# One-2-3-45/One-2-3-45

Hardware: AMD Instinct MI355X
Metric: rays/sec + mesh-extract wall-clock per scene (8x256^2 views, 128^3 vol) (higher is better)
Workload: dtype f32 (matrix products as 3 f16 MFMAs on split operands, fp32 accumulate); 1 GPU; BASELINE config 2: 1 scene/GPU/step (a different seeded scene every step), 8 views 256x256, 128^3 volume, 262144 rays (64+64 samples), mesh grid 256^3; whole scene pass per step; views=8, volume=128, rays=262144, mesh_res=256, parallelism=scenes x1, precision=f16x3

## Files before the change

include/o2345.h:

```cpp
#ifndef O2345_H
#define O2345_H
#include <stddef.h>
#include <stdint.h>
#ifdef __cplusplus
extern "C" {
#endif

const char* o2345_last_error(void);
int o2345_version(void);
size_t o2345_render_io_size(void);
int o2345_render_io_layout(size_t* offsets_host, int n);
const char* o2345_knobs(void);

size_t o2345_costvol_workspace_bytes(int dx, int dy, int dz);
int o2345_costvol_index(const float* proj, int V, int H, int W, int dx, int dy, int dz, float voxel_size,
                        const float* origin_host, int min_views, uint8_t* cnt, int32_t* row_of_voxel, int32_t* coords,
                        int32_t* n_rows_dev, void* workspace, size_t workspace_bytes, void* stream);
int o2345_costvol_gather(const float* feats_nhwc, const float* proj, int V, int H, int W, int C, int dx, int dy, int dz,
                         float voxel_size, const float* origin_host, const uint8_t* cnt, const int32_t* coords,
                         int n_rows, float* out_rows, void* stream);
int o2345_nchw_to_nhwc(const float* in, float* out, int V, int C, int H, int W, void* stream);

int o2345_fpn_level(const float* fine, int c_in, const float* coarse, const float* weight, const float* bias, int V, int H, int W,
                    float* out, void* stream);
// ... 7 lines not shown
size_t o2345_conv2d_x3_weight_floats(int cin, int k);
int o2345_conv2d_pack_weights_x3(const float* w_oihw, int cout, int cin, int k, float* packed, void* stream);
int o2345_conv2d_x3(const float* in, int V, int cin, int Hi, int Wi, int in_pixel_stride, int in_channel_offset, const float* in_scale_shift, float slope,
                    const float* w_packed_x3, const float* bias, int cout, int k, int stride, float* out, const float* gamma, const float* beta, float eps,
                    int abs_gamma, float* out_scale_shift, void* workspace, size_t workspace_bytes, void* stream);
int o2345_fpn_level_act(const float* fine, const float* fine_scale_shift, float slope, int c_in, const float* coarse, const float* weight,
                        const float* bias, int V, int H, int W, float* out, void* stream);
int o2345_scale_shift_act(const float* x, int V, int C, int H, int W, const float* scale_shift, float slope, float* y_nchw, float* y_nhwc,
                          void* stream);
int o2345_visible_count_list(const float* proj, int V, int H, int W, float voxel_size, const float* origin_host,
                             const int32_t* coords, int n, uint8_t* cnt, void* stream);
int o2345_costvol_gather_list(const float* feats_nhwc, const float* proj, int V, int H, int W, int C, float voxel_size,
                              const float* origin_host, const uint8_t* cnt_row, const int32_t* coords, int n_rows,
                              float* out_rows, void* stream);
int o2345_build_index_grid(const int32_t* coords, int n, int ts, int nx, int ny, int nz, int32_t* grid, void* stream);
int o2345_prune_dilate(const float* sdf, const float* mask, int D, float threshold, int radius, uint8_t* out, void* stream);
int o2345_scatter_dense(const float* rows, const int32_t* row_of_voxel, int C, long long nvox, float* dense_cl,
                        float* dense_cf, float* mask, void* stream);

size_t o2345_sparse_downsample_workspace_bytes(int nxc, int nyc, int nzc);
int o2345_sparse_downsample(const int32_t* coords_fine, int n_fine, int ts, int nxc, int nyc, int nzc,
                            int32_t* row_of_cell, int32_t* coords_coarse, int32_t* n_coarse_dev, void* workspace,
                            size_t workspace_bytes, void* stream);
int o2345_sparse_conv3d(int mode, const float* in, int cin, const int32_t* in_grid, int gx, int gy, int gz,
                        const int32_t* out_coords, int n_out, int ts_out, const float* kernel, int cout, float* out,
                        void* stream);
int o2345_sparse_conv_x3_blob_floats(int cin, int cout);
int o2345_sparse_conv3d_x3(int mode, const float* in, int cin, const int32_t* in_grid, int gx, int gy, int gz,
                           const int32_t* out_coords, int n_out, int ts_out, const float* wblob, int cout, int identity_rows, float* out,
                           void* stream);
size_t o2345_bn_workspace_bytes(int C);
int o2345_bn_act_rows(const float* x, int n, int C, const float* gamma, const float* beta, float eps, float slope,
                      int abs_gamma, const float* skip, float* y, float* mean_var_out, void* workspace,
                      size_t workspace_bytes, void* stream);
size_t o2345_abn_workspace_bytes(int C);
int o2345_abn_nchw(const float* x, int V, int C, int H, int W, const float* gamma, const float* beta, float eps,
                   float slope, int abs_gamma, float* y_nchw, float* y_nhwc, void* workspace, size_t workspace_bytes,
                   void* stream);

int o2345_sdf_blob_floats(void);
int o2345_sdf_mlp(int variant, const float* blob, const float* vol_cl, int D, const float* pts, const int32_t* index,
                  const int32_t* n_dev, long long n, int grid_R, float sign, float* out_sdf, float* out_feat,
                  float* out_lat, float* out_grad, void* stream);
int o2345_sdf_mlp_ex(int variant, const float* blob, const float* vol_cl, int D, const float* pts, const int32_t* index,
                     const int32_t* n_dev, long long n, int grid_R, float sign, const float* lat_in, float* out_sdf,
                     float* out_feat, float* out_lat, float* out_grad, void* stream);
int o2345_sdf_mlp_x3(const float* blob, const float* vol_cl, int D, const float* pts, const int32_t* index, const int32_t* n_dev,
                     long long n, int grid_R, float sign, float* out_sdf, void* stream);
int o2345_sdf_grad_x3(const float* blob, const float* vol_cl, int D, const float* pts, const int32_t* index, const int32_t* n_dev,
                      long long n, int grid_R, float sign, float* out_sdf, float* out_grad, void* stream);
int o2345_sdf_grid_tables(const float* tab_axes, const float* bias_lane_order, int grid_R, float* tab_xy, void* stream);
int o2345_sdf_grid_x3(const float* blob, const float* vol_cl, int D, int grid_R, float sign, const float* tab_xy, const float* tab_z,
                      float* out_sdf, void* stream);

int o2345_ray_coarse(const float* rays_o, const float* rays_d, int R, float near, float far, int S, float* z, float* pts,
                     void* stream);
int o2345_ray_coarse_jitter(const float* rays_o, const float* rays_d, int R, float near, float far, int S,
                            const float* t_rand, float* z, float* pts, void* stream);
int o2345_ray_coarse_per_ray(const float* rays_o, const float* rays_d, int R, const float* near_ray, const float* far_ray, int S,
                             const float* t_rand, float* z, float* pts, void* stream);
int o2345_ray_upsample(const float* rays_o, const float* rays_d, int R, const float* z, const float* sdf, int S,
                       float inv_s, const float* maskvol, int D, float* wbuf, int n_imp, float* new_z, float* new_pts,
                       float* new_sdf, int32_t* list, int32_t* count_dev, void* stream);
int o2345_ray_merge(int R, float* z, float* sdf, int S, float* new_z, float* new_sdf, int n_new, void* stream);
int o2345_ray_finalize(const float* rays_o, const float* rays_d, int R, const float* z, int S, float sample_dist,
                       const float* maskvol, int D, float* mid_z, float* dists, float* pts, float* pm, float* sdf,
                       float* grad, float* rgb, int32_t* list, int32_t* count_dev, void* stream);
int o2345_ray_composite(const float* rays_o, const float* rays_d, int R, int S, const float* mid_z, const float* dists,
                        const float* pm, const float* sdf, const float* grad, const float* rgb, const uint8_t* nviews,
                        float inv_s, float alpha_inter_ratio, float background, float* color, float* depth,
                        float* weights, float* cdf, float* weights_sum, float* weights_max, float* depth_var,
                        float* alpha_sum, float* grad_err, uint8_t* color_mask, void* stream);

typedef struct O2345RenderIO {
    const float* sdf_blob;
    const float* color_x3_blob;
    const float* color_mfma_blob;
    const float* vol_cl;
    const float* maskvol;
    const float* cmaps;
    const float* proj;
    const float* cam_pos;
    int D, V, H, W;
    const float* rays_o; const float* rays_d;
    const float* near_ray;
    const float* far_ray;
    const float* query_cam;
    const float* t_rand;
    int R, n_samples, n_importance;
    int sdf_mode;
    int segment_rays;
    float near, far;
    float sample_dist;
    float inv_s, alpha_inter_ratio, background;
    float weight_cull;
    float* mid_z; float* dists; float* pm; float* sdf; float* grad; float* rgb; uint8_t* nviews;
    float* color; float* depth; float* weights; float* cdf; float* weights_sum; float* weights_max; float* depth_var;
    float* alpha_sum; float* grad_err; uint8_t* color_mask;
    float* z_vals;
    float* scalars;
    unsigned long long* color_stats;
} O2345RenderIO;
size_t o2345_list_sort_workspace_bytes(long long n_max, int V);
int o2345_list_sort_by_visibility(const float* pts, const int32_t* list, const int32_t* count_dev, long long n_max, const float* proj, int V, int H, int W,
                                  int32_t* list_out, uint32_t* keys_out, void* workspace, size_t workspace_bytes, void* stream);
size_t o2345_render_workspace_bytes(int R, int n_samples, int n_importance, int V);
// ... 92 lines not shown
```

one-2-3-45_amd/config.py:

```python
import os

PRECISIONS = ("f16x3", "fp32")
PRECISION = os.environ.get("O2345_PRECISION", "f16x3")
if PRECISION not in PRECISIONS:
    raise ValueError(f"O2345_PRECISION must be one of {PRECISIONS}, got {PRECISION!r}")


def sdf_precision(p=None):
    p = PRECISION if p is None else p
    if p not in PRECISIONS:
        raise ValueError(f"unknown precision {p!r}")
    return p


def color_precision(p=None):
    p = PRECISION if p is None else p
    if p not in PRECISIONS:
        raise ValueError(f"unknown precision {p!r}")
    return p


WEIGHT_CULL = float(os.environ.get("O2345_WEIGHT_CULL", "").strip() or 0.0) if "O2345_WEIGHT_CULL" in os.environ else 2.0 ** -24
if not (0.0 <= WEIGHT_CULL < 1.0):
    raise ValueError(f"O2345_WEIGHT_CULL must be in [0, 1), got {WEIGHT_CULL}")


def weight_cull(w=None):
    w = WEIGHT_CULL if w is None else float(w)
    if not (0.0 <= w < 1.0):
        raise ValueError(f"weight_cull must be in [0, 1), got {w}")
    return w


def warm_aten():
    return os.environ.get("O2345_WARM_ATEN", "1") not in ("", "0")


def prepack_resolutions():
    v = os.environ.get("O2345_PREPACK_RESOLUTIONS", "256")
    return tuple(int(x) for x in v.replace(",", " ").split())


def _non_negative_int(name, text):
    t = text.strip()
    if t == "":
        return 0
    if not t.isdigit():
        raise ValueError(f"{name} must be a non-negative integer, got {text!r}")
    return int(t)


MESH_MIN_COMPONENT_FACES = _non_negative_int("O2345_MESH_MIN_COMPONENT_FACES", os.environ.get("O2345_MESH_MIN_COMPONENT_FACES", ""))
MESH_KEEP_LARGEST = _non_negative_int("O2345_MESH_KEEP_LARGEST", os.environ.get("O2345_MESH_KEEP_LARGEST", "")) != 0


def mesh_min_component_faces(n=None):
    if n is None:
        return MESH_MIN_COMPONENT_FACES
    if isinstance(n, bool) or int(n) != n or n < 0:
        raise ValueError(f"min_component_faces must be a non-negative integer, got {n!r}")
    return int(n)


def mesh_keep_largest(k=None):
    return MESH_KEEP_LARGEST if k is None else bool(k)


def _finite_float(name, text, default, ok, what):
    t = text.strip()
    if t == "":
        return default
    try:
        x = float(t)
    except ValueError:
        x = float("nan")
    if not (x == x and abs(x) != float("inf") and ok(x)):
        raise ValueError(f"{name} must be {what}, got {text!r}")
    return x


MESH_SMOOTH_ITERATIONS = _non_negative_int("O2345_MESH_SMOOTH_ITERATIONS", os.environ.get("O2345_MESH_SMOOTH_ITERATIONS", ""))
MESH_SMOOTH_LAMBDA = _finite_float("O2345_MESH_SMOOTH_LAMBDA", os.environ.get("O2345_MESH_SMOOTH_LAMBDA", ""), 0.5, lambda x: 0.0 < x <= 1.0, "in (0, 1]")
MESH_SMOOTH_MU = _finite_float("O2345_MESH_SMOOTH_MU", os.environ.get("O2345_MESH_SMOOTH_MU", ""), -0.53, lambda x: x <= 0.0, "finite and <= 0")
_pin = os.environ.get("O2345_MESH_SMOOTH_PIN_BOUNDARY", "")
MESH_SMOOTH_PIN_BOUNDARY = True if _pin.strip() == "" else _non_negative_int("O2345_MESH_SMOOTH_PIN_BOUNDARY", _pin) != 0
del _pin


def mesh_smooth_iterations(n=None):
    if n is None:
        return MESH_SMOOTH_ITERATIONS
    if isinstance(n, bool) or int(n) != n or n < 0:
        raise ValueError(f"smooth_iterations must be a non-negative integer, got {n!r}")
    return int(n)


def mesh_smooth_lambda(lam=None):
    if lam is None:
        return MESH_SMOOTH_LAMBDA
    return _finite_float("lam", repr(float(lam)), None, lambda x: 0.0 < x <= 1.0, "in (0, 1]")


# ... 93 lines not shown
```

one-2-3-45_amd/csrc/geom_math.h:

```cpp
#pragma once
#include "common.h"

namespace o2345 {

O2345_HD void project_voxel(const float* __restrict__ P, float wx, float wy, float wz, int H, int W,
                            float& gx, float& gy, bool& valid) {
    float x = fmaf(P[2], wz, fmaf(P[1], wy, P[0] * wx)) + P[3];
    float y = fmaf(P[6], wz, fmaf(P[5], wy, P[4] * wx)) + P[7];
    float z = fmaf(P[10], wz, fmaf(P[9], wy, P[8] * wx)) + P[11];
    if (z >= 0.f) z = fmaxf(z, 1e-6f);
    gx = 2.f * (x / z) / (float)(W - 1) - 1.f;
    gy = 2.f * (y / z) / (float)(H - 1) - 1.f;
    valid = (fabsf(gx) <= 1.f) && (fabsf(gy) <= 1.f) && (z > 0.f);
}

struct Taps2D {
    int idx[4];
    float w[4];
};

O2345_HD Taps2D bilinear_taps(float gx, float gy, int H, int W) {
    Taps2D t;
    float ix = (gx + 1.f) / 2.f * (float)(W - 1);
    float iy = (gy + 1.f) / 2.f * (float)(H - 1);
    float x0 = floorf(ix), y0 = floorf(iy);
    float x1 = x0 + 1.f, y1 = y0 + 1.f;
    float wx1 = ix - x0, wx0 = x1 - ix, wy1 = iy - y0, wy0 = y1 - iy;
    bool bx0 = (x0 >= 0.f) && (x0 <= (float)(W - 1)), bx1 = (x1 >= 0.f) && (x1 <= (float)(W - 1));
    bool by0 = (y0 >= 0.f) && (y0 <= (float)(H - 1)), by1 = (y1 >= 0.f) && (y1 <= (float)(H - 1));
    int xi0 = (int)fminf(fmaxf(x0, 0.f), (float)(W - 1)), xi1 = (int)fminf(fmaxf(x1, 0.f), (float)(W - 1));
    int yi0 = (int)fminf(fmaxf(y0, 0.f), (float)(H - 1)), yi1 = (int)fminf(fmaxf(y1, 0.f), (float)(H - 1));
    t.idx[0] = yi0 * W + xi0; t.w[0] = (bx0 && by0) ? wx0 * wy0 : 0.f;
    t.idx[1] = yi0 * W + xi1; t.w[1] = (bx1 && by0) ? wx1 * wy0 : 0.f;
    t.idx[2] = yi1 * W + xi0; t.w[2] = (bx0 && by1) ? wx0 * wy1 : 0.f;
    t.idx[3] = yi1 * W + xi1; t.w[3] = (bx1 && by1) ? wx1 * wy1 : 0.f;
    return t;
}

struct Taps3D {
    int ix[2], iy[2], iz[2];
    float fx[2], fy[2], fz[2];
    bool ok;
};

O2345_HD Taps3D trilinear_ref_taps(float px, float py, float pz, int D) {
    Taps3D t;
    const float s = (float)(D - 1);
    float ix = (px + 1.f) / 2.f * s, iy = (py + 1.f) / 2.f * s, iz = (pz + 1.f) / 2.f * s;
    const float Df = (float)D;
    t.ok = (ix > 0.f) && (ix < Df) && (iy > 0.f) && (iy < Df) && (iz > 0.f) && (iz < Df);
    float x0 = floorf(ix), y0 = floorf(iy), z0 = floorf(iz);
    t.fx[0] = (x0 + 1.f) - ix; t.fx[1] = ix - x0;
    t.fy[0] = (y0 + 1.f) - iy; t.fy[1] = iy - y0;
    t.fz[0] = (z0 + 1.f) - iz; t.fz[1] = iz - z0;
    auto cl = [s](float v) { return (int)fminf(fmaxf(v, 0.f), s); };
    t.ix[0] = cl(x0); t.ix[1] = cl(x0 + 1.f);
    t.iy[0] = cl(y0); t.iy[1] = cl(y0 + 1.f);
    t.iz[0] = cl(z0); t.iz[1] = cl(z0 + 1.f);
    return t;
}

O2345_HD int nearest_index(float g, int D) {
    float i = nearbyintf(((g + 1.f) * (float)D - 1.f) / 2.f);
    return (i >= 0.f && i <= (float)(D - 1)) ? (int)i : -1;
}

O2345_HD int nearest_voxel(float px, float py, float pz, int D) {
    int x = nearest_index(px, D), y = nearest_index(py, D), z = nearest_index(pz, D);
    return (x < 0 || y < 0 || z < 0) ? -1 : (x * D + y) * D + z;
}

struct Axis2 {
    int i[2];
    float w[2];
};
O2345_HD Axis2 axis_taps_zeros(float g, int D) {
    Axis2 a;
    float s = (float)(D - 1);
    float f = (g + 1.f) / 2.f * s;
    float f0 = floorf(f), f1 = f0 + 1.f;
    a.w[0] = (f0 >= 0.f && f0 <= s) ? (f1 - f) : 0.f;
    a.w[1] = (f1 >= 0.f && f1 <= s) ? (f - f0) : 0.f;
    a.i[0] = (int)fminf(fmaxf(f0, 0.f), s);
    a.i[1] = (int)fminf(fmaxf(f1, 0.f), s);
    return a;
}

}
```

one-2-3-45_amd/csrc/sdf_common.h:

```cpp
#pragma once
#include "common.h"
#include "geom_math.h"
#include "pe_math.h"
#include "split_f16.h"

namespace o2345 {

constexpr int ST0 = 20;
constexpr int ST1 = 72;
constexpr int STB = 64;
constexpr int OFF_A0 = 0;
constexpr int OFF_A1 = OFF_A0 + 4 * ST0 * 64;
constexpr int OFF_A2 = OFF_A1 + 4 * ST1 * 64;
constexpr int OFF_A1T = OFF_A2 + 4 * ST1 * 64;
constexpr int OFF_A0T = OFF_A1T + 5 * STB * 64;
constexpr int OFF_MISC = OFF_A0T + 2 * STB * 64;
constexpr int MISC_B0 = 0, MISC_B1 = 128, MISC_B2 = 256, MISC_W2H = 384, MISC_W2L = 512, MISC_SIZE = 528;
constexpr int BLOB_F32_FLOATS = OFF_MISC + MISC_SIZE;
constexpr int OFFX_MISC = BLOB_F32_FLOATS;
constexpr int STX0 = 3;
constexpr int STH1 = 9;
constexpr int STHB = 8;
constexpr int OFFX_A0 = OFFX_MISC + MISC_SIZE;
static_assert(OFFX_A0 % 4 == 0, "the float4 staging and the b128 buffer loads of the split-f16 sections need 16-byte alignment");
// ... 51 lines not shown
    m[0] = fmaxf(a[0], 0.f); m[1] = fmaxf(a[1], 0.f);
    return __builtin_elementwise_fma(l, f32x2{0.00693147180559945309f, 0.00693147180559945309f}, m);
}

__device__ __forceinline__ f32x2 softplus100_pair(f32x2 a, f32x2& dsig) {
    const f32x2 t = a * 144.269504088896340736f;
    f32x2 e;
    e[0] = __builtin_amdgcn_exp2f(-__builtin_fabsf(t[0]));
    e[1] = __builtin_amdgcn_exp2f(-__builtin_fabsf(t[1]));
    const f32x2 u = e + 1.f;
    f32x2 l, m, ru;
    l[0] = __builtin_amdgcn_logf(u[0]); l[1] = __builtin_amdgcn_logf(u[1]);
    ru[0] = __builtin_amdgcn_rcpf(u[0]); ru[1] = __builtin_amdgcn_rcpf(u[1]);
    m[0] = fmaxf(a[0], 0.f); m[1] = fmaxf(a[1], 0.f);
    f32x2 q = ru - 0.5f;
    q[0] = __builtin_copysignf(q[0], a[0]); q[1] = __builtin_copysignf(q[1], a[1]);
    dsig = q + 0.5f;
    return __builtin_elementwise_fma(l, f32x2{0.00693147180559945309f, 0.00693147180559945309f}, m);
}

constexpr float SOFTPLUS_INV_SCALE = 0.00693147180559945309f;
__device__ __forceinline__ f32x2 softplus_t_pair(f32x2 t) {
    f32x2 e;
    e[0] = __builtin_amdgcn_exp2f(-__builtin_fabsf(t[0]));
    e[1] = __builtin_amdgcn_exp2f(-__builtin_fabsf(t[1]));
    const f32x2 u = e + 1.f;
    f32x2 l, m;
    l[0] = __builtin_amdgcn_logf(u[0]); l[1] = __builtin_amdgcn_logf(u[1]);
    m[0] = fmaxf(t[0], 0.f); m[1] = fmaxf(t[1], 0.f);
    return l + m;
}
__device__ __forceinline__ f32x2 softplus_t_pair(f32x2 t, f32x2& dsig) {
    f32x2 e;
    e[0] = __builtin_amdgcn_exp2f(-__builtin_fabsf(t[0]));
    e[1] = __builtin_amdgcn_exp2f(-__builtin_fabsf(t[1]));
    const f32x2 u = e + 1.f;
    f32x2 l, m, ru;
    l[0] = __builtin_amdgcn_logf(u[0]); l[1] = __builtin_amdgcn_logf(u[1]);
    ru[0] = __builtin_amdgcn_rcpf(u[0]); ru[1] = __builtin_amdgcn_rcpf(u[1]);
    m[0] = fmaxf(t[0], 0.f); m[1] = fmaxf(t[1], 0.f);
    f32x2 q = ru - 0.5f;
    q[0] = __builtin_copysignf(q[0], t[0]); q[1] = __builtin_copysignf(q[1], t[1]);
    dsig = q + 0.5f;
    return l + m;
}
__device__ __forceinline__ float softplus_t_d(float t) {
    return __builtin_amdgcn_rcpf(1.f + __builtin_amdgcn_exp2f(-t));
}

__device__ __forceinline__ float softplus100_d(float a) {
    return __builtin_amdgcn_rcpf(1.f + __builtin_amdgcn_exp2f(a * -144.269504088896340736f));
}

__device__ __forceinline__ float lin11(int i, int R) {
    const float step = 2.f / (float)(R - 1);
    return (i < R / 2) ? fmaf(step, (float)i, -1.f) : fmaf(-step, (float)(R - 1 - i), 1.f);
}


struct TilePoint {
    long long slot;
    float px, py, pz;
    int ix, iy, iz;
};
__device__ __forceinline__ TilePoint sdf_tile_point(const SdfArgs& a, bool use_pts, long long i, bool live) {
    TilePoint p;
    p.slot = live ? (a.index ? (long long)a.index[i] : i) : 0;
    p.ix = p.iy = p.iz = 0;
    if (use_pts) {
        p.px = live ? a.pts[p.slot * 3 + 0] : 0.f; p.py = live ? a.pts[p.slot * 3 + 1] : 0.f; p.pz = live ? a.pts[p.slot * 3 + 2] : 0.f;
    } else {
        const int R = a.R;
        const unsigned us = (unsigned)p.slot, uR = (unsigned)R;
        const unsigned uq = us / uR;
        p.iz = (int)(us - uq * uR); p.ix = (int)(uq / uR); p.iy = (int)(uq - (uq / uR) * uR);
        p.px = lin11(p.ix, R); p.py = lin11(p.iy, R); p.pz = lin11(p.iz, R);
    }
    return p;
}

__device__ __forceinline__ void latent_voxel(const float* vol_cl, int D, const Taps3D& tp, int dx, int dy, int dz, int h, float (&v)[8]) {
    const size_t vox = ((size_t)tp.ix[dx] * D + tp.iy[dy]) * D + tp.iz[dz];
    const float4* p4 = reinterpret_cast<const float4*>(vol_cl + vox * 16 + 8 * h);
    const float4 v0 = p4[0], v1 = p4[1];
    v[0] = v0.x; v[1] = v0.y; v[2] = v0.z; v[3] = v0.w; v[4] = v1.x; v[5] = v1.y; v[6] = v1.z; v[7] = v1.w;
}

__device__ __forceinline__ void latent_gather(const float* vol_cl, int D, float px, float py, float pz, int h, bool live, float (&lat)[8]) {
#pragma unroll
    for (int c = 0; c < 8; ++c) lat[c] = 0.f;
    const Taps3D tp = trilinear_ref_taps(px, py, pz, D);
    if (tp.ok && live) {
#pragma unroll
        for (int dx = 0; dx < 2; ++dx)
#pragma unroll
            for (int dy = 0; dy < 2; ++dy)
#pragma unroll
                for (int dz = 0; dz < 2; ++dz) {
                    float v[8];
                    latent_voxel(vol_cl, D, tp, dx, dy, dz, h, v);
                    const float w = tp.fz[dz] * tp.fy[dy] * tp.fx[dx];
#pragma unroll
                    for (int c = 0; c < 8; ++c) lat[c] = fmaf(v[c], w, lat[c]);
                }
    }
}

__device__ __forceinline__ void latent_grad(const float* vol_cl, int D, float px, float py, float pz, int h, bool live, const float (&gl)[8], float (&gx)[3]) {
    const Taps3D tp = trilinear_ref_taps(px, py, pz, D);
    if (tp.ok && live) {
        const float half_span = (float)(D - 1) * 0.5f;
// ... 152 lines not shown
```

one-2-3-45_amd/csrc/sdf_mlp_x3.hip:

```cpp
#include "sdf_common.h"

namespace o2345 {

template <int NB, int NST, int B0 = 0, int B1 = NB>
__device__ __forceinline__ void mma_x3_part(f32x16 (&acc)[NB], const float4* A, int lane, int step, const Split8& b) {
    h16x8 ahi[B1 - B0], alo[B1 - B0];
#pragma unroll
    for (int ob = B0; ob < B1; ++ob) {
        ahi[ob - B0] = __builtin_bit_cast(h16x8, A[((ob * NST + step) * 2 + 0) * 64 + lane]);
        alo[ob - B0] = __builtin_bit_cast(h16x8, A[((ob * NST + step) * 2 + 1) * 64 + lane]);
    }
    mfma_x3<B1 - B0>(acc + B0, ahi, alo, b);
    __builtin_amdgcn_sched_barrier(0);
}
template <int NB, int NST>
__device__ __forceinline__ void mma_x3(f32x16 (&acc)[NB], const float4* A, int lane, int step, const Split8& b) {
    if constexpr (NB > 4) {
        mma_x3_part<NB, NST, 0, 3>(acc, A, lane, step, b);
        mma_x3_part<NB, NST, 3, NB>(acc, A, lane, step, b);
    } else {
        mma_x3_part<NB, NST, 0, NB>(acc, A, lane, step, b);
    }
}

// ... 132 lines not shown
        acc_from_bias(acc, misc, MISC_B1, h);
#pragma unroll
        for (int s = 0; s < 8; ++s) mma_x3<4, STH1>(acc, A1, lane, s, hb[s]);
        mma_x3<4, STH1>(acc, A1, lane, 8, latx);
        AReg<2> tcur = a_fetch<2, STHB>(rs, OFFX_A1T, lane, 3, 0);
        Split8 g1x[8];
        const float yh = softplus_split_grad(acc, misc, h, g1x, m1);
        float y0 = fmaf(yh, SOFTPLUS_INV_SCALE, ylat);
        y0 += __shfl_xor(y0, 32);
        y0 += misc[MISC_B2];
        if (live && h == 0) a.out_sdf[slot] = a.sign * y0;
        __syncthreads();
        f32x16 g[5];
        acc_zero(g);
#pragma unroll
        for (int s = 0; s < 8; ++s) {
            mfma_x3<2>(g + 3, tcur.hi, tcur.lo, g1x[s]);
            __builtin_amdgcn_sched_barrier(0);
            if (s + 1 < 8) tcur = a_fetch<2, STHB>(rs, OFFX_A1T, lane, 3, s + 1);
            mma_x3_part<5, STHB, 0, 3>(g, A1T, lane, s, g1x[s]);
        }
        f32x16 gp[2];
        acc_zero(gp);
#pragma unroll
        for (int nb = 0; nb < 4; ++nb) {
            const AReg<2> ta = a_fetch<2, STHB>(rs, OFFX_A0T, lane, 0, 2 * nb);
            __builtin_amdgcn_sched_barrier(0);
            f32x16 a0r[1];
            acc_from_bias(a0r, misc, MISC_B0 + nb * 32, h);
#pragma unroll
            for (int s = 0; s < STX0; ++s) mma_x3_part<1, STX0, 0, 1>(a0r, A0 + nb * STX0 * 2 * 64, lane, s, pex[s]);
            const AReg<2> tb = a_fetch<2, STHB>(rs, OFFX_A0T, lane, 0, 2 * nb + 1);
            __builtin_amdgcn_sched_barrier(0);
            float gv[16];
#pragma unroll
            for (int r = 0; r < 16; ++r) gv[r] = g[nb][r] * softplus_t_d(a0r[0][r]);
            mfma_x3<2>(gp, ta.hi, ta.lo, split8<MIXLO>(gv, 0, m1));
            mfma_x3<2>(gp, tb.hi, tb.lo, split8<MIXLO>(gv, 8, m1));
            __builtin_amdgcn_sched_barrier(0);
        }
        float gx[3], gl[8];
        pe_chain_rule(gp, h, pe_at, gx);
#pragma unroll
        for (int t = 0; t < 8; ++t) gl[t] = g[4][t] + misc[MISC_W2L + 8 * h + t];
        latent_grad(a.vol_cl, a.D, px, py, pz, h, live, gl, gx);
#pragma unroll
        for (int d = 0; d < 3; ++d) gx[d] += __shfl_xor(gx[d], 32);
        if (live && h == 0 && a.out_grad) {
            a.out_grad[slot * 3 + 0] = gx[0]; a.out_grad[slot * 3 + 1] = gx[1]; a.out_grad[slot * 3 + 2] = gx[2];
        }
    }
}

}

using namespace o2345;

extern "C" {

static int sdf_x3_check(const char* what, bool pointers, int D, bool has_pts, int grid_R) {
    O2345_REQUIRE(pointers, "%s: null pointer", what);
    O2345_REQUIRE(D >= 2, "%s: bad volume side %d", what, D);
    O2345_REQUIRE(has_pts || (grid_R >= 2 && grid_R <= 1600), "%s: need points or a grid resolution in [2, 1600]", what);
    return 0;
}

int o2345_sdf_grad_x3(const float* blob, const float* vol_cl, int D, const float* pts, const int32_t* index, const int32_t* n_dev,
                      long long n, int grid_R, float sign, float* out_sdf, float* out_grad, void* stream) {
    if (const int rc = sdf_x3_check("sdf_grad_x3", blob && vol_cl && out_sdf && out_grad, D, pts, grid_R)) return rc;
    if (n <= 0 && !n_dev) return 0;
    const SdfArgs a{blob, vol_cl, D, pts, index, n_dev, n, grid_R, sign, out_sdf, nullptr, nullptr, out_grad, nullptr};
    return sdf_launch<k_sdf_grad_x3, LDSX_GRAD_FLOATS>("sdf_grad_x3", a, stream);
}

int o2345_sdf_mlp_x3(const float* blob, const float* vol_cl, int D, const float* pts, const int32_t* index, const int32_t* n_dev,
                     long long n, int grid_R, float sign, float* out_sdf, void* stream) {
    if (const int rc = sdf_x3_check("sdf_mlp_x3", blob && vol_cl && out_sdf, D, pts, grid_R)) return rc;
    if (n <= 0 && !n_dev) return 0;
    const SdfArgs a{blob, vol_cl, D, pts, index, n_dev, n, grid_R, sign, out_sdf, nullptr, nullptr, nullptr, nullptr, nullptr, nullptr};
    return sdf_launch<k_sdf_mlp_x3<false>, LDSX_MLP_FLOATS>("sdf_mlp_x3", a, stream);
}

__global__ __launch_bounds__(128) void k_sdf_tab_xy(const float* __restrict__ axes , const float* __restrict__ bias , int R,
                                                     float* __restrict__ tab_xy) {
    const int c = threadIdx.x, ix = blockIdx.x / R, iy = blockIdx.x % R;
    tab_xy[(size_t)blockIdx.x * 128 + c] = (float)((double)axes[(size_t)ix * 128 + c] + (double)axes[((size_t)R + iy) * 128 + c] + (double)bias[c]);
}

int o2345_sdf_grid_tables(const float* tab_axes, const float* bias_lane_order, int grid_R, float* tab_xy, void* stream) {
    O2345_REQUIRE(tab_axes && bias_lane_order && tab_xy && grid_R >= 2 && grid_R <= 1600, "sdf_grid_tables: bad arguments");
    hipLaunchKernelGGL(k_sdf_tab_xy, dim3(grid_R * grid_R), dim3(128), 0, (hipStream_t)stream, tab_axes, bias_lane_order, grid_R, tab_xy);
    return check_launch("sdf_grid_tables");
}

int o2345_sdf_grid_x3(const float* blob, const float* vol_cl, int D, int grid_R, float sign, const float* tab_xy, const float* tab_z, float* out_sdf,
                      void* stream) {
    if (const int rc = sdf_x3_check("sdf_grid_x3", blob && vol_cl && out_sdf && tab_xy && tab_z, D, false, grid_R)) return rc;
    const long long n = (long long)grid_R * grid_R * grid_R;
    const SdfArgs a{blob, vol_cl, D, nullptr, nullptr, nullptr, n, grid_R, sign, out_sdf, nullptr, nullptr, nullptr, nullptr, tab_xy, tab_z};
    return sdf_launch<k_sdf_mlp_x3<true>, LDSX_MLP_FLOATS>("sdf_grid_x3", a, stream);
}

}

namespace o2345 {
int preload_sdf_mlp_x3() {
    hipFuncAttributes at;
    return (int)hipFuncGetAttributes(&at, (const void*)(k_sdf_grad_x3));
}
}
```

one-2-3-45_amd/ops.py:

```python
import ctypes
import functools
import threading

import numpy as np
import torch

from . import _lib, config, mesh_io
from ._lib import check


def _stream():
    return ctypes.c_void_p(torch.cuda.current_stream().cuda_stream)


def _first_cuda_tensor(objs):
    for o in objs:
        if torch.is_tensor(o):
            if o.is_cuda:
                return o
        elif isinstance(o, dict):
            t = _first_cuda_tensor(o.values())
            if t is not None:
                return t
    return None
# ... 302 lines not shown

@_on_device
def sparse_conv3d_x3(mode, x, in_grid, in_cells, out_coords, ts_out, wblob, cout, identity_rows=False):
    n_out, cin = out_coords.shape[0], x.shape[1]
    out = torch.empty(n_out, cout, dtype=torch.float32, device=x.device)
    if n_out == 0 or x.shape[0] == 0:
        return out.zero_()
    if identity_rows and (int(mode) != 0 or n_out != x.shape[0]):
        raise ValueError(f"sparse_conv3d_x3: identity_rows needs mode 0 and one output row per input row (mode {mode}, {n_out} vs {x.shape[0]} rows)")
    check(_lib.lib().o2345_sparse_conv3d_x3(int(mode), _p(x), cin, _p(in_grid, torch.int32), in_cells[0], in_cells[1], in_cells[2],
                                            _p(out_coords, torch.int32), n_out, int(ts_out), _p(wblob), int(cout), int(bool(identity_rows)), _p(out),
                                            _stream()), "sparse_conv3d_x3")
    return out


@_on_device
def bn_act_rows(x, gamma, beta, eps=1e-5, slope=0.0, abs_gamma=False, skip=None, want_stats=False):
    L = _lib.lib()
    n, C = x.shape
    y = torch.empty_like(x)
    if n == 0:
        return (y, torch.zeros(2, C, device=x.device)) if want_stats else y
    wsb = L.o2345_bn_workspace_bytes(C)
    ws = _workspace(wsb, x.device, "bn")
    mv = torch.empty(2, C, dtype=torch.float32, device=x.device) if want_stats else None
    check(L.o2345_bn_act_rows(_p(x), n, C, _p(gamma), _p(beta), float(eps), float(slope), int(abs_gamma), _p(skip), _p(y),
                              _p(mv), _p(ws, torch.uint8), wsb, _stream()), "bn_act_rows")
    return (y, mv) if want_stats else y


@_on_device
def abn_nchw(x, gamma, beta, eps=1e-5, slope=0.01, abs_gamma=True, want_nchw=True, want_nhwc=False):
    L = _lib.lib()
    V, C, H, W = x.shape
    wsb = L.o2345_abn_workspace_bytes(C)
    ws = _workspace(wsb, x.device, "abn")
    y1 = torch.empty_like(x) if want_nchw else None
    y2 = torch.empty(V, H, W, C, dtype=torch.float32, device=x.device) if want_nhwc else None
    check(L.o2345_abn_nchw(_p(x), V, C, H, W, _p(gamma), _p(beta), float(eps), float(slope), int(abs_gamma), _p(y1), _p(y2),
                           _p(ws, torch.uint8), wsb, _stream()), "abn_nchw")
    return y1, y2


@_on_device
def sdf_grid_tables(tab_axes, bias_lane_order):
    R = tab_axes.shape[1]
    tab_xy = torch.empty(R * R, 128, dtype=torch.float32, device=tab_axes.device)
    check(_lib.lib().o2345_sdf_grid_tables(_p(tab_axes), _p(bias_lane_order), R, _p(tab_xy), _stream()), "sdf_grid_tables")
    return tab_xy, tab_axes[2]


@_on_device
def sdf_mlp(blob, vol_cl, pts=None, variant=0, grid_R=0, sign=1.0, index=None, n_dev=None, want_lat=False, out=None, lat_in=None,
            precision=None, grid_tables=None):
    precision = config.sdf_precision(precision)
    D = vol_cl.shape[0]
    dev = vol_cl.device
    if pts is not None:
        P = pts.shape[0]
    else:
        P = int(grid_R) ** 3
    n = P if index is None else index.shape[0]
    res = out or {}
    if "sdf" not in res:
        res["sdf"] = torch.empty(P, dtype=torch.float32, device=dev)
    if variant == 1 and "feat" not in res:
        res["feat"] = torch.empty(P, 128, dtype=torch.float32, device=dev)
    if variant == 2 and "grad" not in res:
        res["grad"] = torch.empty(P, 3, dtype=torch.float32, device=dev)
    if want_lat and "lat" not in res:
        res["lat"] = torch.empty(P, 16, dtype=torch.float32, device=dev)
    if P == 0 or (n == 0 and n_dev is None):
        return res
    if precision == "f16x3" and variant == 0 and not want_lat and lat_in is None:
        if grid_tables is not None and pts is None and index is None and n_dev is None:
            tab_xy, tab_z = grid_tables
            if tuple(tab_xy.shape) != (int(grid_R) ** 2, 128) or tuple(tab_z.shape) != (int(grid_R), 128):
                raise ValueError(f"sdf_mlp: grid tables were built for another resolution than {grid_R}")
            check(_lib.lib().o2345_sdf_grid_x3(_p(blob), _p(vol_cl), D, int(grid_R), float(sign), _p(tab_xy), _p(tab_z), _p(res["sdf"]), _stream()),
                  "sdf_grid_x3")
            return res
        check(_lib.lib().o2345_sdf_mlp_x3(_p(blob), _p(vol_cl), D, _p(pts), _p(index, torch.int32), _p(n_dev, torch.int32), n, int(grid_R),
                                          float(sign), _p(res["sdf"]), _stream()), "sdf_mlp_x3")
        return res
    if precision == "f16x3" and variant == 2 and not want_lat and lat_in is None:
        check(_lib.lib().o2345_sdf_grad_x3(_p(blob), _p(vol_cl), D, _p(pts), _p(index, torch.int32), _p(n_dev, torch.int32), n, int(grid_R),
                                           float(sign), _p(res["sdf"]), _p(res["grad"]), _stream()), "sdf_grad_x3")
        return res
    check(_lib.lib().o2345_sdf_mlp_ex(int(variant), _p(blob), _p(vol_cl), D, _p(pts), _p(index, torch.int32), _p(n_dev, torch.int32),
                                      n, int(grid_R), float(sign), _p(lat_in), _p(res["sdf"]), _p(res.get("feat")), _p(res.get("lat")),
                                      _p(res.get("grad")), _stream()), "sdf_mlp")
    return res


@_on_device
def pack_color_maps(feat_nchw, color_nchw):
    V, _, H, W = feat_nchw.shape
    out = torch.empty(V, H, W, 64, dtype=torch.float32, device=feat_nchw.device)
    check(_lib.lib().o2345_pack_color_maps(_p(feat_nchw), _p(color_nchw), V, H, W, _p(out), _stream()), "pack_color_maps")
    return out


@_on_device
def camera_terms(intrinsics, w2cs):
    V = intrinsics.shape[0]
    if tuple(intrinsics.shape) != (V, 3, 3) or tuple(w2cs.shape) != (V, 4, 4):
        raise ValueError(f"camera_terms: intrinsics [V,3,3] and w2cs [V,4,4] expected, got {tuple(intrinsics.shape)}, {tuple(w2cs.shape)}")
    proj = torch.empty(V, 3, 4, dtype=torch.float32, device=w2cs.device)
    cam = torch.empty(V, 3, dtype=torch.float32, device=w2cs.device)
    check(_lib.lib().o2345_camera_terms(_p(_f(intrinsics)), _p(_f(w2cs)), V, _p(proj), _p(cam), _stream()), "camera_terms")
    return proj, cam


def color_stats_buffer(device):
    return torch.zeros(4, dtype=torch.int64, device=device)


def color_stats_read(buf):
    out = [int(x) for x in buf.cpu().tolist()]
    return dict(pairs_pooling=out[0], pairs_network=out[1], tiles=out[2], tiles_all_views=out[3])


@_on_device
def color_points(blob, vol_cl, maskvol, cmaps, proj, cam_pos, pts, query_cam=None, normals=None, index=None, n_dev=None,
                 want_nviews=True, mfma="x3", stats=None):
    if mfma is False or mfma is None:
        raise ValueError("color_points: the pure-VALU colour kernel was removed in ABI 2.0; pass mfma='x3' (split-f16) or mfma=True (fp32 MFMA)")
    V, H, W, _ = cmaps.shape
    P = pts.shape[0]
    n = P if index is None else index.shape[0]
    rgb = torch.zeros(P, 3, dtype=torch.float32, device=pts.device)
    nv = torch.zeros(P, dtype=torch.uint8, device=pts.device) if want_nviews else None
    if P == 0 or (n == 0 and n_dev is None):
        return rgb, nv
    L = _lib.lib()
    fn = L.o2345_color_points_x3 if mfma == "x3" else L.o2345_color_points_mfma
    check(fn(_p(blob), _p(vol_cl), _p(maskvol), vol_cl.shape[0], _p(cmaps), _p(proj), _p(cam_pos),
             V, H, W, _p(pts), _p(index, torch.int32), _p(n_dev, torch.int32), n, _p(query_cam),
             _p(normals), _p(rgb), _p(nv, torch.uint8), _p(stats, torch.int64), _stream()), "color_points")
    return rgb, nv


@_on_device
def project_features(vol_cl, maskvol, cmaps, proj, cam_pos, pts, query_cam=None, normals=None):
    V, H, W, _ = cmaps.shape
# ... 535 lines not shown
```

one-2-3-45_amd/pipeline.py:

```python
import numpy as np
import torch
import torch.nn.functional as F

from . import config, ops, weights
from .costreg import CostRegNet
from .featurenet import ConvBnReLU, FeatureNet, fused_pyramid, set_precision


def _load_checked(module, sd, what):
    res = module.load_state_dict(sd, strict=False)
    missing = [k for k in res.missing_keys if not ("running_" in k or "num_batches_tracked" in k)]
    if missing or res.unexpected_keys:
        raise KeyError(f"{what}: checkpoint does not match (missing {missing}, unexpected {list(res.unexpected_keys)})")


class SceneWeights:

    def __init__(self, device, seed=0, sdf=None, color_sd=None, costreg_sd=None, variance=0.2, sdf_precision=None, color_precision=None):
        self.device = device
        sdf_precision = config.sdf_precision(sdf_precision)
        color_precision = config.color_precision(color_precision)
        self.color_precision = color_precision
        self.sdf_precision = sdf_precision
        with torch.random.fork_rng(devices=[]):
            torch.manual_seed(seed)
            self.featurenet = set_precision(FeatureNet().to(device), color_precision)
            self.compress = set_precision(ConvBnReLU(56, 16).to(device), color_precision)
        self.sdfW = sdf or weights.init_sdf_weights(seed)
        self.color_sd = color_sd or weights.init_color_state_dict(seed)
        self.costreg_sd = costreg_sd or weights.init_costreg_state_dict(seed)
        t = lambda a: torch.from_numpy(a).to(device)
        self.sdf_blob = t(weights.pack_sdf_blob(self.sdfW))
        self.color_mblob = t(weights.pack_color_mfma_blob(self.color_sd))
        self.color_xblob = t(weights.pack_color_x3_blob(self.color_sd))
        self.costreg = CostRegNet(self.costreg_sd, device, precision=color_precision)
        self._grid_tabs = {}
        self.variance = float(variance)
        self.inv_s = float(np.clip(np.exp(10.0 * variance), 1e-6, 1e6))

    def grid_tables(self, resolution):
        if self.sdf_precision != "f16x3":
            return None
        R = int(resolution)
        if R not in self._grid_tabs:
            axes, bias = weights.sdf_grid_tables(self.sdfW, R)
            dev = self.sdf_blob.device
            self._grid_tabs[R] = ops.sdf_grid_tables(torch.from_numpy(axes).to(dev), torch.from_numpy(bias).to(dev))
        return self._grid_tabs[R]

    @classmethod
    def from_state_dicts(cls, device, sdf_network_sd, rendering_network_sd, variance, featurenet_sd=None, sdf_precision=None, color_precision=None):
        t = lambda v: torch.as_tensor(np.asarray(v.detach().cpu() if torch.is_tensor(v) else v))
        sd = {k: t(v) for k, v in sdf_network_sd.items()}
        costreg = {k[len("sparse_costreg_net."):]: v for k, v in sd.items() if k.startswith("sparse_costreg_net.")}
        self = cls(device, seed=0, sdf=weights.sdf_weights_from_state_dict(sd, "sdf_layer."),
                   color_sd={k: t(v).numpy() for k, v in rendering_network_sd.items()}, costreg_sd=costreg, variance=float(variance),
                   sdf_precision=sdf_precision, color_precision=color_precision)
        comp = {k[len("compress_layer."):]: v for k, v in sd.items() if k.startswith("compress_layer.")}
        _load_checked(self.compress, comp, "compress_layer")
        if featurenet_sd is not None:
            _load_checked(self.featurenet, {k: t(v) for k, v in featurenet_sd.items()}, "pyramid_feature_network")
        return self


    @staticmethod
    def _read_checkpoint(path, names, allow_pickle=None):
        import os
        if allow_pickle is None:
            allow_pickle = os.environ.get("O2345_ALLOW_PICKLE", "0") not in ("", "0")
        try:
            ck = torch.load(path, map_location="cpu", weights_only=True)
        except Exception as e:
            if not allow_pickle:
                raise RuntimeError(f"o2345 SceneWeights.from_checkpoint: {path!r} does not load with the restricted unpickler ({type(e).__name__}: {e}); "
                                   "pass allow_pickle=True (or O2345_ALLOW_PICKLE=1) only for a checkpoint you trust -- the full unpickler runs code "
                                   "from the file") from e
            import warnings
            warnings.warn(f"o2345: loading {path!r} with the FULL unpickler (allow_pickle): code in the file is executed")
            ck = torch.load(path, map_location="cpu", weights_only=False)
        return {n: {k: v for k, v in ck[n].items() if torch.is_tensor(v) and v.is_floating_point()} for n in names}

    @classmethod
    def from_checkpoint(cls, device, path, broadcast=False, sdf_precision=None, color_precision=None, allow_pickle=None):
        import torch.distributed as dist
        from . import sharding
        names = ("sdf_network_lod0", "rendering_network_lod0", "variance_network_lod0", "pyramid_feature_network")
        if broadcast and not (dist.is_available() and dist.is_initialized()):
            raise RuntimeError("SceneWeights.from_checkpoint(broadcast=True) needs an initialised torch.distributed process group (sharding.init)")
        state = None
        if not broadcast or dist.get_rank() == 0:
            try:
                state = cls._read_checkpoint(path, names, allow_pickle)
            except Exception as e:
                if not broadcast:
                    raise
                state = e
        if broadcast:
            state = sharding.broadcast_state_dicts(state, device)
        return cls.from_state_dicts(device, state["sdf_network_lod0"], state["rendering_network_lod0"], state["variance_network_lod0"]["variance"],
                                    featurenet_sd=state["pyramid_feature_network"], sdf_precision=sdf_precision, color_precision=color_precision)

# ... 20 lines not shown
def camera_terms(intrinsics, w2cs):
    return ops.camera_terms(intrinsics, w2cs)


@torch.no_grad()
def render(wt, vol, proj, cam_pos, rays_o, rays_d, near, far, query_cam, n_samples=64, n_importance=64, want_z=False, t_rand=None):
    scene = dict(sdf_blob=wt.sdf_blob, vol_cl=vol["vol_cl"], maskvol=vol["maskvol"],
                 cmaps=vol["cmaps"], proj=proj, cam_pos=cam_pos, color_mfma_blob=wt.color_mblob,
                 sdf_precision=wt.sdf_precision, color_precision=wt.color_precision,
                 color_x3_blob=wt.color_xblob)
    return ops.render_rays(scene, rays_o, rays_d, near, far, n_samples, n_importance, wt.inv_s, 1.0, 1.0, query_cam, want_z, t_rand=t_rand)


@torch.no_grad()
def render_scene_split(wt, imgs, affine_mats, origin, D, voxel_size, proj, cam_pos, rays_o, rays_d, near, far, query_cam, src=0,
                       keys=("color", "depth", "weights_sum", "color_mask"), **render_kw):
    from . import sharding as sh
    dev = rays_o.device
    imgs = sh.broadcast_tensor(imgs, src=src, device=dev)
    vol = build_volume(wt, imgs, affine_mats, origin, D, voxel_size)
    rank, world = (torch.distributed.get_rank(), torch.distributed.get_world_size()) if torch.distributed.is_initialized() else (0, 1)
    lo, hi, per = sh.ray_block(rays_o.shape[0], rank, world)
    R_all = rays_o.shape[0]
    per_ray = lambda a, b: {k: (v[a:b].contiguous() if torch.is_tensor(v) and v.dim() >= 1 and v.shape[0] == R_all else v)
                            for k, v in render_kw.items()}
    if hi > lo:
        o = render(wt, vol, proj, cam_pos, rays_o[lo:hi].contiguous(), rays_d[lo:hi].contiguous(), near, far, query_cam, **per_ray(lo, hi))
        block = {k: o[k] for k in keys}
    else:
        o = render(wt, vol, proj, cam_pos, rays_o[:1].contiguous(), rays_d[:1].contiguous(), near, far, query_cam, **per_ray(0, 1))
        block = {k: o[k][:0] for k in keys}
    return sh.gather_ray_blocks(block, rays_o.shape[0], per, device=dev), vol


def _index_to_world(idx, resolution):
    return idx / (resolution - 1.0) * 2.0 - 1.0


def _colours_at(wt, vol, proj, cam_pos, pts):
    g = ops.sdf_mlp(wt.sdf_blob, vol["vol_cl"], pts, variant=2, precision=wt.sdf_precision)["grad"]
    x3 = wt.color_precision == "f16x3"
    rgb, _ = ops.color_points(wt.color_xblob if x3 else wt.color_mblob, vol["vol_cl"], vol["maskvol"], vol["cmaps"], proj, cam_pos, pts, normals=g,
                              want_nviews=False, mfma="x3" if x3 else True)
    return rgb, g


def _mesh_fields(wt, vol, proj, cam_pos, resolution, min_component_faces=None, keep_largest=None, info=None, smooth_iterations=None, decimate_cell=None,
                 project_iterations=None, texture=None):
    min_faces, largest = config.mesh_min_component_faces(min_component_faces), config.mesh_keep_largest(keep_largest)
    smooth = config.mesh_smooth_iterations(smooth_iterations)
    cell = config.mesh_decimate_cell(decimate_cell)
    project = config.mesh_project_iterations(project_iterations)
    prec = wt.sdf_precision
    u = ops.sdf_mlp(wt.sdf_blob, vol["vol_cl"], None, variant=0, grid_R=resolution, sign=-1.0, precision=prec, grid_tables=wt.grid_tables(resolution))["sdf"]
    u = u.view(resolution, resolution, resolution)
    verts_idx, tris = ops.marching_cubes(u, 0.0)
    cc = None
    if min_faces or largest:
        verts_idx, tris, _, cc = ops.mesh_filter_components(verts_idx, tris, min_faces, largest)
    dec = None
    if cell:
        verts_idx, tris, _, dec = ops.mesh_decimate(verts_idx, tris, cell)
    pro = None
    if project:
        verts_idx, pro = ops.mesh_project(wt.sdf_blob, vol["vol_cl"], verts_idx, resolution, project, max_move=config.mesh_project_max_move(None, cell),
                                          precision=prec)
    if info is not None:
        info["components"], info["components_kept"] = (cc["components"], cc["components_kept"]) if cc else (None, None)
        info["decimate"] = dec
        info["project"] = pro
    verts = _index_to_world(verts_idx, resolution)
    pts = verts.to(torch.float32).contiguous()
    if pts.shape[0] == 0:
        return verts, verts_idx, tris, torch.zeros(0, 3, device=pts.device), u, None
    rgb, g = _colours_at(wt, vol, proj, cam_pos, pts)
    if texture is not None and tris.shape[0]:
        tpts, tworld, tstats = ops.mesh_texture_points(verts_idx, tris, texture["texel"], resolution, validate=False)
        tpro = None
        if project:
            tpts, tpro = ops.mesh_project(wt.sdf_blob, vol["vol_cl"], tpts, resolution, project, max_move=config.mesh_project_max_move(None, cell), precision=prec)
            tworld = _index_to_world(tpts, resolution).to(torch.float32).contiguous()
        trgb, _ = _colours_at(wt, vol, proj, cam_pos, tworld)
        texture.update(rgb=trgb, stats=tstats, project=tpro, layout=ops.mesh_io.texture_layout(tris.shape[0], texture["texel"]))
    if smooth:
        verts_idx = ops.mesh_smooth(verts_idx, tris, smooth)
        verts = _index_to_world(verts_idx, resolution)
    return verts, verts_idx, tris, rgb, u, g


def _texture_block(texture):
    if not texture or "layout" not in texture:
        return None
    L = texture["layout"]
    return {"width": L["width"], "height": L["height"], "texel": L["texel"], "texels": L["texels"]}


@torch.no_grad()
def extract_mesh(wt, vol, proj, cam_pos, resolution, return_index_verts=False, min_component_faces=None, keep_largest=None, smooth_iterations=None,
                 decimate_cell=None, project_iterations=None):
    verts, verts_idx, tris, rgb, u, _ = _mesh_fields(wt, vol, proj, cam_pos, resolution, min_component_faces, keep_largest, smooth_iterations=smooth_iterations,
                                                     decimate_cell=decimate_cell, project_iterations=project_iterations)
    return (verts_idx if return_index_verts else verts), tris, rgb, u


@torch.no_grad()
def export_mesh_ply(path, wt, vol, proj, cam_pos, resolution, scale_mat=None, trans_mat=None, min_component_faces=None, keep_largest=None,
                    smooth_iterations=None, decimate_cell=None, project_iterations=None):
# ... 59 lines not shown
```

Baseline: 4.533 million rays/s.

## Skip SDF MLP on grid tiles outside the mask, fill from cached background

Adds a sparse path for the 256^3 mesh-extraction SDF grid. A pre-pass marks 32-point tiles whose trilinear taps all hit empty mask voxels and writes a cached, weight-only background SDF there. It then compacts the remaining active tiles into an index list, and only those run through the f16x3 MLP kernel. The background is the MLP evaluated on a zero feature volume; it is built on the second extraction at a resolution and kept, at the cost of extra memory (up to 64MB at R=256). This relies on masked-out voxels having zero features, and adds an atomic compaction pass.

```diff
diff --git a/include/o2345.h b/include/o2345.h
--- a/include/o2345.h
+++ b/include/o2345.h
@@ -83,6 +83,9 @@
 int o2345_sdf_grid_tables(const float* tab_axes, const float* bias_lane_order, int grid_R, float* tab_xy, void* stream);
 int o2345_sdf_grid_x3(const float* blob, const float* vol_cl, int D, int grid_R, float sign, const float* tab_xy, const float* tab_z,
                       float* out_sdf, void* stream);
+size_t o2345_sdf_grid_sparse_workspace_bytes(int grid_R);
+int o2345_sdf_grid_sparse_x3(const float* blob, const float* vol_cl, const float* maskvol, int D, int grid_R, float sign, const float* tab_xy,
+                             const float* tab_z, const float* background, float* out_sdf, void* workspace, size_t workspace_bytes, void* stream);
 
 int o2345_ray_coarse(const float* rays_o, const float* rays_d, int R, float near, float far, int S, float* z, float* pts,
                      void* stream);
diff --git a/one-2-3-45_amd/config.py b/one-2-3-45_amd/config.py
--- a/one-2-3-45_amd/config.py
+++ b/one-2-3-45_amd/config.py
@@ -48,6 +48,20 @@
     if not t.isdigit():
         raise ValueError(f"{name} must be a non-negative integer, got {text!r}")
     return int(t)
+
+
+_gb = os.environ.get("O2345_GRID_BACKGROUND_MB", "")
+GRID_BACKGROUND_MB = 256 if _gb.strip() == "" else _non_negative_int("O2345_GRID_BACKGROUND_MB", _gb)
+del _gb
+
+
+def grid_background_mb():
+    return GRID_BACKGROUND_MB
+
+
+def grid_background_allowed(resolution):
+    n = int(resolution) ** 3
+    return n < 2 ** 31 and 4 * n <= grid_background_mb() << 20
 
 
 MESH_MIN_COMPONENT_FACES = _non_negative_int("O2345_MESH_MIN_COMPONENT_FACES", os.environ.get("O2345_MESH_MIN_COMPONENT_FACES", ""))
diff --git a/one-2-3-45_amd/csrc/geom_math.h b/one-2-3-45_amd/csrc/geom_math.h
--- a/one-2-3-45_amd/csrc/geom_math.h
+++ b/one-2-3-45_amd/csrc/geom_math.h
@@ -60,6 +60,30 @@
     return t;
 }
 
+O2345_HD float lin11(int i, int R) {
+    const float step = 2.f / (float)(R - 1);
+    return (i < R / 2) ? fmaf(step, (float)i, -1.f) : fmaf(-step, (float)(R - 1 - i), 1.f);
+}
+
+O2345_HD bool grid_point_active(long long slot, int R, int D, const float* __restrict__ maskvol) {
+    const unsigned us = (unsigned)slot, uR = (unsigned)R, uq = us / uR;
+    const int iz = (int)(us - uq * uR), ix = (int)(uq / uR), iy = (int)(uq - (uq / uR) * uR);
+    const Taps3D tp = trilinear_ref_taps(lin11(ix, R), lin11(iy, R), lin11(iz, R), D);
+    bool kept = false;
+    for (int dx = 0; dx < 2; ++dx)
+        for (int dy = 0; dy < 2; ++dy)
+            for (int dz = 0; dz < 2; ++dz) kept |= maskvol[((size_t)tp.ix[dx] * D + tp.iy[dy]) * D + tp.iz[dz]] != 0.f;
+    return tp.ok && kept;
+}
+
+constexpr int GRID_TILE = 32;
+O2345_HD bool grid_tile_active(long long tile, int R, int D, const float* __restrict__ maskvol) {
+    const long long n = (long long)R * R * R, lo = tile * GRID_TILE, hi = lo + GRID_TILE < n ? lo + GRID_TILE : n;
+    for (long long s = lo; s < hi; ++s)
+        if (grid_point_active(s, R, D, maskvol)) return true;
+    return false;
+}
+
 O2345_HD int nearest_index(float g, int D) {
     float i = nearbyintf(((g + 1.f) * (float)D - 1.f) / 2.f);
     return (i >= 0.f && i <= (float)(D - 1)) ? (int)i : -1;
diff --git a/one-2-3-45_amd/csrc/sdf_common.h b/one-2-3-45_amd/csrc/sdf_common.h
--- a/one-2-3-45_amd/csrc/sdf_common.h
+++ b/one-2-3-45_amd/csrc/sdf_common.h
@@ -127,11 +127,6 @@
     return __builtin_amdgcn_rcpf(1.f + __builtin_amdgcn_exp2f(a * -144.269504088896340736f));
 }
 
-__device__ __forceinline__ float lin11(int i, int R) {
-    const float step = 2.f / (float)(R - 1);
-    return (i < R / 2) ? fmaf(step, (float)i, -1.f) : fmaf(-step, (float)(R - 1 - i), 1.f);
-}
-
 
 struct TilePoint {
     long long slot;
diff --git a/one-2-3-45_amd/csrc/sdf_mlp_x3.hip b/one-2-3-45_amd/csrc/sdf_mlp_x3.hip
--- a/one-2-3-45_amd/csrc/sdf_mlp_x3.hip
+++ b/one-2-3-45_amd/csrc/sdf_mlp_x3.hip
@@ -208,6 +208,38 @@
     }
 }
 
+constexpr int GRID_CHUNK_TILES = 256;
+constexpr size_t GRID_WS_HEAD = 256;
+static_assert(GRID_TILE == 32 && GRID_CHUNK_TILES % 64 == 0, "a tile is one half of a wave, as in k_sdf_mlp_x3");
+__global__ __launch_bounds__(GRID_CHUNK_TILES) void k_grid_active_tiles(const float* __restrict__ maskvol, int D, int R, const float* __restrict__ background,
+                                                                        float sign, float* __restrict__ out, int32_t* __restrict__ index, int32_t* n_active) {
+    __shared__ int s_active[GRID_CHUNK_TILES], s_list[GRID_CHUNK_TILES], s_wave[GRID_CHUNK_TILES / 64 + 1], s_base;
+    const long long n = (long long)R * R * R;
+    const long long tile0 = (long long)blockIdx.x * GRID_CHUNK_TILES;
+    const int lane = threadIdx.x & 63, wave = threadIdx.x >> 6, half = lane >> 5;
+    for (int it = 0; it < GRID_CHUNK_TILES / 8; ++it) {
+        const int t = it * 8 + wave * 2 + half;
+        const long long slot = (tile0 + t) * GRID_TILE + (lane & 31);
+        const bool live = slot < n;
+        const unsigned long long b = __ballot(live && grid_point_active(slot, R, D, maskvol));
+        const bool tile_active = (half ? (b >> 32) : (b & 0xffffffffull)) != 0;
+        if (live && !tile_active) out[slot] = sign * background[slot];
+        if ((lane & 31) == 0) s_active[t] = tile_active;
+    }
+    __syncthreads();
+    const bool mine = s_active[threadIdx.x] != 0;
+    int total;
+    const int pos = block_prefix<GRID_CHUNK_TILES / 64>(mine, s_wave, total);
+    if (mine) s_list[pos] = threadIdx.x;
+    if (threadIdx.x == 0) s_base = total ? atomicAdd(n_active, total * GRID_TILE) : 0;
+    __syncthreads();
+    const int base = s_base;
+    for (int e = threadIdx.x; e < total * GRID_TILE; e += GRID_CHUNK_TILES) {
+        const long long slot = (tile0 + s_list[e >> 5]) * GRID_TILE + (e & 31);
+        index[base + e] = (int32_t)(slot < n ? slot : n - 1);
+    }
+}
+
 }
 
 using namespace o2345;
@@ -257,6 +289,31 @@
     return sdf_launch<k_sdf_mlp_x3<true>, LDSX_MLP_FLOATS>("sdf_grid_x3", a, stream);
 }
 
+size_t o2345_sdf_grid_sparse_workspace_bytes(int grid_R) {
+    if (grid_R < 2 || (long long)grid_R * grid_R * grid_R >= (1ll << 31)) return 0;
+    const long long ntiles = ((long long)grid_R * grid_R * grid_R + GRID_TILE - 1) / GRID_TILE;
+    return GRID_WS_HEAD + (size_t)ntiles * GRID_TILE * sizeof(int32_t);
+}
+
+int o2345_sdf_grid_sparse_x3(const float* blob, const float* vol_cl, const float* maskvol, int D, int grid_R, float sign, const float* tab_xy,
+                             const float* tab_z, const float* background, float* out_sdf, void* workspace, size_t workspace_bytes, void* stream) {
+    if (const int rc = sdf_x3_check("sdf_grid_sparse_x3", blob && vol_cl && maskvol && background && out_sdf && tab_xy && tab_z && workspace, D, false, grid_R))
+        return rc;
+    const long long n = (long long)grid_R * grid_R * grid_R;
+    O2345_REQUIRE(n < (1ll << 31), "sdf_grid_sparse_x3: grid_R^3 must stay below 2^31 (got %d)", grid_R);
+    O2345_REQUIRE(workspace_bytes >= o2345_sdf_grid_sparse_workspace_bytes(grid_R) && ((uintptr_t)workspace & 15) == 0,
+                  "sdf_grid_sparse_x3: workspace too small or misaligned");
+    int32_t* n_active = reinterpret_cast<int32_t*>(workspace);
+    int32_t* index = reinterpret_cast<int32_t*>(static_cast<char*>(workspace) + GRID_WS_HEAD);
+    O2345_HIP(hipMemsetAsync(n_active, 0, sizeof(int32_t), (hipStream_t)stream));
+    const long long ntiles = (n + GRID_TILE - 1) / GRID_TILE;
+    hipLaunchKernelGGL(k_grid_active_tiles, dim3(cdiv(ntiles, GRID_CHUNK_TILES)), dim3(256), 0, (hipStream_t)stream, maskvol, D, grid_R, background, sign,
+                       out_sdf, index, n_active);
+    if (const int rc = check_launch("sdf_grid_sparse_x3 (active tiles)")) return rc;
+    const SdfArgs a{blob, vol_cl, D, nullptr, index, n_active, n, grid_R, sign, out_sdf, nullptr, nullptr, nullptr, nullptr, tab_xy, tab_z};
+    return sdf_launch<k_sdf_mlp_x3<true>, LDSX_MLP_FLOATS>("sdf_grid_sparse_x3", a, stream);
+}
+
 }
 
 namespace o2345 {
diff --git a/one-2-3-45_amd/ops.py b/one-2-3-45_amd/ops.py
--- a/one-2-3-45_amd/ops.py
+++ b/one-2-3-45_amd/ops.py
@@ -378,7 +378,7 @@
 
 @_on_device
 def sdf_mlp(blob, vol_cl, pts=None, variant=0, grid_R=0, sign=1.0, index=None, n_dev=None, want_lat=False, out=None, lat_in=None,
-            precision=None, grid_tables=None):
+            precision=None, grid_tables=None, maskvol=None, grid_background=None):
     precision = config.sdf_precision(precision)
     D = vol_cl.shape[0]
     dev = vol_cl.device
@@ -396,6 +396,10 @@
         res["grad"] = torch.empty(P, 3, dtype=torch.float32, device=dev)
     if want_lat and "lat" not in res:
         res["lat"] = torch.empty(P, 16, dtype=torch.float32, device=dev)
+    sparse = maskvol is not None or grid_background is not None
+    if sparse and not (maskvol is not None and grid_background is not None and precision == "f16x3" and variant == 0 and not want_lat and lat_in is None
+                       and grid_tables is not None and pts is None and index is None and n_dev is None):
+        raise ValueError("sdf_mlp: maskvol and grid_background come together and with grid_tables only (f16x3, variant 0, the whole lattice)")
     if P == 0 or (n == 0 and n_dev is None):
         return res
     if precision == "f16x3" and variant == 0 and not want_lat and lat_in is None:
@@ -403,6 +407,16 @@
             tab_xy, tab_z = grid_tables
             if tuple(tab_xy.shape) != (int(grid_R) ** 2, 128) or tuple(tab_z.shape) != (int(grid_R), 128):
                 raise ValueError(f"sdf_mlp: grid tables were built for another resolution than {grid_R}")
+            if sparse:
+                if maskvol.numel() != D ** 3 or grid_background.numel() != P or P >= 2 ** 31:
+                    raise ValueError(f"sdf_mlp: maskvol [{D}^3] and grid_background [{grid_R}^3 < 2^31] expected, got {maskvol.numel()} and "
+                                     f"{grid_background.numel()} elements")
+                L = _lib.lib()
+                wsb = L.o2345_sdf_grid_sparse_workspace_bytes(int(grid_R))
+                ws = _workspace(wsb, dev, "sdf_grid_sparse")
+                check(L.o2345_sdf_grid_sparse_x3(_p(blob), _p(vol_cl), _p(maskvol), D, int(grid_R), float(sign), _p(tab_xy), _p(tab_z), _p(grid_background),
+                                                 _p(res["sdf"]), _p(ws, torch.uint8), wsb, _stream()), "sdf_grid_sparse_x3")
+                return res
             check(_lib.lib().o2345_sdf_grid_x3(_p(blob), _p(vol_cl), D, int(grid_R), float(sign), _p(tab_xy), _p(tab_z), _p(res["sdf"]), _stream()),
                   "sdf_grid_x3")
             return res
@@ -417,6 +431,12 @@
                                       n, int(grid_R), float(sign), _p(lat_in), _p(res["sdf"]), _p(res.get("feat")), _p(res.get("lat")),
                                       _p(res.get("grad")), _stream()), "sdf_mlp")
     return res
+
+
+def sdf_grid_active_points(device):
+    with torch.cuda.device(device):
+        ws = _ws_cache.get(("sdf_grid_sparse", str(torch.device(device)), torch.cuda.current_stream(device).cuda_stream))
+    return None if ws is None else int(ws[:4].view(torch.int32).item())
 
 
 @_on_device
diff --git a/one-2-3-45_amd/pipeline.py b/one-2-3-45_amd/pipeline.py
--- a/one-2-3-45_amd/pipeline.py
+++ b/one-2-3-45_amd/pipeline.py
@@ -35,6 +35,8 @@
         self.color_xblob = t(weights.pack_color_x3_blob(self.color_sd))
         self.costreg = CostRegNet(self.costreg_sd, device, precision=color_precision)
         self._grid_tabs = {}
+        self._grid_bg = {}
+        self._grid_extractions = {}
         self.variance = float(variance)
         self.inv_s = float(np.clip(np.exp(10.0 * variance), 1e-6, 1e6))
 
@@ -47,6 +49,19 @@
             dev = self.sdf_blob.device
             self._grid_tabs[R] = ops.sdf_grid_tables(torch.from_numpy(axes).to(dev), torch.from_numpy(bias).to(dev))
         return self._grid_tabs[R]
+
+    def grid_background(self, resolution):
+        R = int(resolution)
+        if self.sdf_precision != "f16x3" or not config.grid_background_allowed(R):
+            return None
+        if R not in self._grid_bg:
+            seen = self._grid_extractions.get(R, 0)
+            self._grid_extractions[R] = seen + 1
+            if seen == 0:
+                return None
+            empty = torch.zeros(2, 2, 2, 16, dtype=torch.float32, device=self.sdf_blob.device)
+            self._grid_bg[R] = ops.sdf_mlp(self.sdf_blob, empty, None, variant=0, grid_R=R, sign=1.0, precision="f16x3", grid_tables=self.grid_tables(R))["sdf"]
+        return self._grid_bg[R]
 
     @classmethod
     def from_state_dicts(cls, device, sdf_network_sd, rendering_network_sd, variance, featurenet_sd=None, sdf_precision=None, color_precision=None):
@@ -173,7 +188,9 @@
     cell = config.mesh_decimate_cell(decimate_cell)
     project = config.mesh_project_iterations(project_iterations)
     prec = wt.sdf_precision
-    u = ops.sdf_mlp(wt.sdf_blob, vol["vol_cl"], None, variant=0, grid_R=resolution, sign=-1.0, precision=prec, grid_tables=wt.grid_tables(resolution))["sdf"]
+    bg = wt.grid_background(resolution)
+    u = ops.sdf_mlp(wt.sdf_blob, vol["vol_cl"], None, variant=0, grid_R=resolution, sign=-1.0, precision=prec, grid_tables=wt.grid_tables(resolution),
+                    maskvol=vol["maskvol"] if bg is not None else None, grid_background=bg)["sdf"]
     u = u.view(resolution, resolution, resolution)
     verts_idx, tris = ops.marching_cubes(u, 0.0)
     cc = None
```

Result: faster. 4.598 million rays/s, median of 6 (+1.4%).
